# Qualcomm-AI-research/FP8-quantization

Measured on AMD Instinct MI355X. Metric: FP8 quant+dequant Gelems/sec, higher is better.
Workload: dtype f32; 1 GPU; conv1-shaped weights [2097152,3,7,7] fp32 per GPU, per-channel E5M2 quantize+dequantize, fixed ranges from current_minmax (BASELINE config 2, synthetic NxCxKxK scale-up); elements_per_gpu=308281344, parallelism=1 GPU

## Files before the change

### fp8-quantization_amd/csrc/fp8q_device.h

```cpp
#pragma once
#include <hip/hip_runtime.h>
#include <stdint.h>

#include "fp8q_tables.h"

namespace fp8q {

typedef float vf4 __attribute__((ext_vector_type(4)));
typedef float vf4u __attribute__((ext_vector_type(4), aligned(4)));

constexpr int kBlock = 256;
constexpr int kLutMax = 130;

struct QFmt {
    float M;
    float two_E;
    float l_c;
    float qthr;
    int sign_bits;
    int pmax;
};

struct __attribute__((aligned(16))) Chan {
    float maxv, minv, bias;
// ... 91 lines not shown

__device__ __forceinline__ void stage_fast_tab(double *dst)
{
    for (int i = threadIdx.x; i < kFastTabSize; i += kBlock) dst[i] = kFastTab[i];
}

__device__ __forceinline__ float scale_exact(const Chan &c, float ls, float M)
{
    if (__builtin_expect(!(fabsf(c.bias) < __builtin_inff()), 0))
        return c.bias != c.bias ? c.bias : (c.bias > 0.0f ? 0.0f : __builtin_inff());
    const float k = ls - M;
    const float e = k - c.bias;
    const double d = (double)k - c.bias_d;
    const double delta = (double)e - d;
    const double u = delta * 0.69314718055994530942;
    const double t = fma(u, 0.5 * u, u);
    const double s = fma(c.g, t, c.g);
    return (float)ldexp(s, (int)k - c.bi);
}

__device__ __forceinline__ float2 lut_entry(const Chan &c, int p, float M)
{
    if (p == 0) return make_float2(__builtin_nanf(""), __builtin_nanf(""));
    const float k = (float)p - M;
    const float e = k - c.bias;
    float s;
    if ((k - e) == c.bias && c.pthr >= 0.0f)
        s = ldexpf(c.m0, (int)k - c.bi);
    else
        s = scale_exact(c, (float)p, M);
    return make_float2(s, __builtin_amdgcn_rcpf(s));
}

__device__ __forceinline__ void lut_row(float2 *lr, const Chan &c, const QFmt &f)
{
    const float k1 = 1.0f - f.M, kp = (float)f.pmax - f.M;
    const bool lin = c.pthr >= 0.0f && (k1 - (k1 - c.bias)) == c.bias && (kp - (kp - c.bias)) == c.bias;
    lr[0] = make_float2(__builtin_nanf(""), __builtin_nanf(""));
    if (lin) {
        const int j0 = (int)k1 - c.bi - 1;
        for (int p = 1; p <= f.pmax; ++p) {
            const float sc = ldexpf(c.m0, j0 + p);
            lr[p] = make_float2(sc, __builtin_amdgcn_rcpf(sc));
        }
    } else {
        for (int p = 1; p <= f.pmax; ++p) lr[p] = lut_entry(c, p, f.M);
    }
}

__device__ __forceinline__ void lut_part(float2 *lr, const Chan &c, const QFmt &f, int sub, int step)
{
    const float k1 = 1.0f - f.M, kp = (float)f.pmax - f.M;
    const bool lin = c.pthr >= 0.0f && (k1 - (k1 - c.bias)) == c.bias && (kp - (kp - c.bias)) == c.bias;
    if (sub == 0) lr[0] = make_float2(__builtin_nanf(""), __builtin_nanf(""));
    if (lin) {
        const int j0 = (int)k1 - c.bi - 1;
        for (int p = sub ? sub : step; p <= f.pmax; p += step) {
            const float sc = ldexpf(c.m0, j0 + p);
            lr[p] = make_float2(sc, __builtin_amdgcn_rcpf(sc));
        }
    } else {
        for (int p = sub ? sub : step; p <= f.pmax; p += step) lr[p] = lut_entry(c, p, f.M);
    }
}

struct ChanLite {
    float maxv, minv, bias, pthr;
};

__device__ __forceinline__ ChanLite lite(const Chan &c)
{
    ChanLite l;
    l.maxv = c.maxv;
    l.minv = c.minv;
    l.bias = c.bias;
    l.pthr = c.pthr;
    return l;
}

__device__ __forceinline__ ChanLite lite_of(const float4 h)
{
    ChanLite l;
    l.maxv = h.x;
    l.minv = h.y;
    l.bias = h.z;
    l.pthr = h.w;
// ... 41 lines not shown
        any |= rk[j];
    }
    if (__builtin_expect(any, 0)) {
#pragma unroll
        for (int j = 0; j < N; ++j)
            if (rk[j]) y[j] = quant_exact(v[j], c.maxv, c.minv, c.bias, lut, pmaxf);
    }
#pragma unroll
    for (int j = 0; j < N; ++j) v[j] = y[j];
}

__device__ __forceinline__ float quant_one(float x, const ChanLite &c, const float2 *lut, float pmaxf,
                                           float qthr)
{
    bool risky;
    float y = quant_fast(x, c, lut, pmaxf, qthr, risky);
    if (__builtin_expect(risky, 0)) y = quant_exact(x, c.maxv, c.minv, c.bias, lut, pmaxf);
    return y;
}

__device__ __forceinline__ float quant_direct(float x, const Chan &c, float M)
{
    const float xc = __builtin_amdgcn_fmed3f(x, c.minv, c.maxv);
    const float a = fabsf(xc);
    const float v = __builtin_amdgcn_logf(a) + c.bias;
    float fl = floorf(v);
    const float fr = v - fl;
    const bool risky = __builtin_amdgcn_classf(x, 0x90) | (fabsf(fr - 0.5f) > c.pthr) | (c.pthr < 0.0f);
    if (__builtin_expect(risky, 0)) fl = floorf(log2_tab(a, kFastTab) + c.bias);
    const float ls = fmaxf(fl, 1.0f);
    const float s = scale_exact(c, ls, M);
    const float y = rintf(xc / s) * s;
    return (x != x) ? x : y;
}

__device__ __forceinline__ uint32_t code_of_r(float r, float ls, int M, int sign_shift)
{
    if (__builtin_expect(!(fabsf(r) <= (float)(2u << M)), 0)) return 0u;
    const uint32_t ri = (uint32_t)fabsf(r);
    const uint32_t m2 = 1u << M;
    uint32_t e = (uint32_t)ls, f = ri - m2;
    if (ri < m2) {
        e = 0u;
        f = ri;
    } else if (ri == 2u * m2) {
        e += 1u;
        f = 0u;
    }
    const uint32_t sign = sign_shift >= 0 ? ((__float_as_uint(r) >> 31) << sign_shift) : 0u;
    return sign | (e << M) | f;
}

__device__ __forceinline__ uint32_t encode_one(float x, const ChanLite &c, const float2 *lut, float pmaxf,
                                               float qthr, int M, int sign_shift)
{
    const float xc = __builtin_amdgcn_fmed3f(x, c.minv, c.maxv);
    const float v = __builtin_amdgcn_logf(fabsf(xc)) + c.bias;
    float fl = floorf(v);
    const float fr = v - fl;
    float ls = __builtin_amdgcn_fmed3f(fl, 1.0f, pmaxf);
    float2 t = lut[(int)ls];
    float q0 = xc * t.y;
    float r = rintf(q0);
    const bool risky = __builtin_amdgcn_classf(x, 0x93) | (fabsf(fr - 0.5f) > c.pthr) |
                       (fabsf(q0 - r) > qthr) | (c.pthr < 0.0f);
    if (__builtin_expect(risky, 0)) {
// ... 183 lines not shown
```

### fp8-quantization_amd/csrc/fp8q_rows.h

```cpp
#pragma once
#include "fp8q_common.h"

namespace {

constexpr int kModeQuant = 0, kModeFused = 1, kModeMinMax = 2;
constexpr int kModeEncode = 3, kModeDecode = 4;

struct TileArgs {
    int inner;
    int rows;
    int lut_stride;
    int group;
    int coaligned;
    uint32_t magic;
    uint32_t lmagic;
};

__device__ __forceinline__ ChanLite lite_lds(const Chan *c)
{
    const float4 h = *reinterpret_cast<const float4 *>(c);
    ChanLite l;
    l.maxv = h.x;
    l.minv = h.y;
    l.bias = h.z;
    l.pthr = h.w;
    return l;
}

constexpr int kChunkElems = 4096, kChunkGroups = 1024, kFlatMaxCh = 8;
constexpr int kFlatFusedMaxInner = 256;

struct FlatArgs {
    int inner;
    int rpc;
    int nch;
    int lut_stride;
    int group;
    int tail;
    uint32_t magic;
// ... 59 lines not shown
```

### fp8-quantization_amd/csrc/fp8q_rows.hip

```cpp
#include "fp8q_rows.h"

namespace {

template <int MODE, bool LUT, bool NT>
__global__ void __launch_bounds__(kBlock, 4)
k_rows_direct(const float *__restrict__ x, float *__restrict__ y, int64_t C,
              const float *__restrict__ maxval, float *row_min, float *row_max, float *maxval_out,
              QFmt f, TileArgs a, FoldArgs fa)
{
    extern __shared__ __attribute__((aligned(16))) unsigned char smem[];
    const int Rmax = a.rows;
    float *rowmv = reinterpret_cast<float *>(smem);
    float4 *patch = reinterpret_cast<float4 *>(rowmv + ((Rmax + 3) & ~3));
    Chan *chans = reinterpret_cast<Chan *>(patch + Rmax);
    float2 *lut = reinterpret_cast<float2 *>(chans + Rmax);
    const int tid = threadIdx.x;
    constexpr int BS = kBlock;
    const int G = a.group, rpp = BS / G;
    const int sub = tid & (G - 1), slot = tid / G;
    const int inner = a.inner, inner4 = inner & ~3;
    const float pmaxf = (float)f.pmax;
    __shared__ double ftab_lds[kFastTabSize];
    const double *ftab = ftab_lds;
    if (MODE != kModeMinMax)
// ... 90 lines not shown
            for (int j0 = tid; j0 < nvec; j0 += BS * U) {
                vf4 v[U];
#pragma unroll
                for (int u = 0; u < U; ++u)
                    if (j0 + u * BS < nvec) v[u] = ld16u<NT>(xt + head + (j0 + u * BS) * 4);
#pragma unroll
                for (int u = 0; u < U; ++u) {
                    const int j = j0 + u * BS;
                    if (j >= nvec) break;
                    const int o = head + j * 4;
                    const int ch = div_small((uint32_t)o, a.magic);
                    const int b = inner - (o - ch * inner);
                    float e[4] = {v[u].x, v[u].y, v[u].z, v[u].w};
                    if (LUT) {
                        quant_group<4>(e, lite_lds(chans + ch), lut + ch * a.lut_stride, pmaxf, f.qthr);
                    } else {
                        const Chan c = chans[ch];
#pragma unroll
                        for (int q = 0; q < 4; ++q) e[q] = quant_direct(e[q], c, f.M);
                    }
                    if (b < 4) {
                        const float4 pt = patch[ch];
                        e[3] = b == 3 ? pt.x : (b == 2 ? pt.y : pt.z);
                        if (b < 3) e[2] = b == 2 ? pt.x : pt.y;
                        if (b < 2) e[1] = pt.x;
                    }
                    st16u<NT>(yt + o, vf4{e[0], e[1], e[2], e[3]});
                }
            }
        }
    }
}

template <int MODE, bool NT>
__global__ void __launch_bounds__(kBlock, 4)
k_rows_flat(const float *__restrict__ x, float *__restrict__ y, const float *__restrict__ maxval,
            float *row_min, float *row_max, float *maxval_out, QFmt f, FlatArgs a)
{
    extern __shared__ __attribute__((aligned(16))) unsigned char smem[];
    __shared__ double ftab[kFastTabSize];
    const int Rt = a.rpc * a.nch;
    ChunkInfo *cinfo = reinterpret_cast<ChunkInfo *>(smem);
    float4 *patch = reinterpret_cast<float4 *>(cinfo + kFlatMaxCh);
    float4 *chl = patch + Rt;
    float2 *lut = reinterpret_cast<float2 *>(chl + Rt);
    float *rowmv = reinterpret_cast<float *>(lut + Rt * a.lut_stride);
    const int tid = threadIdx.x;
    const int inner = a.inner;
    const int64_t G = gridDim.x;
    const float pmaxf = (float)f.pmax;
    for (int i = tid; i < kFastTabSize; i += kBlock) ftab[i] = kFastTab[i];

    for (int64_t c0 = blockIdx.x; c0 < a.nchunks; c0 += G * a.nch) {
        int nct = 1;
        while (nct < a.nch && c0 + nct * G < a.nchunks) ++nct;
        const int nlr = nct * a.rpc;
        __syncthreads();
        if (tid < nct) {
            const int64_t c = c0 + tid * G;
            const int64_t elo = c * kChunkElems;
            const int64_t rem = a.nvec * 4 - elo;
            ChunkInfo ci;
            ci.len = rem < kChunkElems ? (int)rem : kChunkElems;
            ci.tail = (c == a.nchunks - 1) ? a.tail : 0;
            ci.row_lo = elo / inner;
            ci.phase = (int)(elo - ci.row_lo * inner);
            ci.nrows = (ci.phase + ci.len + ci.tail - 1) / inner + 1;
            ci.pad[0] = ci.pad[1] = 0;
            cinfo[tid] = ci;
        }
        __syncthreads();
// ... 217 lines not shown
}

__device__ __forceinline__ ChunkInfo stage_geometry_next(const ChunkInfo &cur, int64_t cn, uint32_t adv, const FlatArgs &a)
{
    ChunkInfo ci;
    const int64_t elo = cn * kChunkElems;
    const int64_t rem = a.nvec * 4 - elo;
    ci.len = rem < kChunkElems ? (int)rem : kChunkElems;
    ci.tail = (cn == a.nchunks - 1) ? a.tail : 0;
    const uint32_t t = (uint32_t)cur.phase + adv;
    const uint32_t q = (uint32_t)div_small(t, a.magic);
    ci.row_lo = cur.row_lo + q;
    ci.phase = (int)(t - q * (uint32_t)a.inner);
    ci.nrows = div_small((uint32_t)(ci.phase + ci.len + ci.tail - 1), a.magic) + 1;
    ci.pad[0] = ci.nrows * a.inner - ci.phase - ci.len;
    ci.pad[1] = 0;
    return ci;
}

constexpr int kStageU = 4;

template <bool NT>
__device__ __forceinline__ void stage_load_body(const float *x, int64_t c, const FlatArgs &a, vf4 (&v)[kStageU])
{
    const int64_t elo = c * kChunkElems;
    const int64_t rem = a.nvec * 4 - elo;
    const int ng = (rem < kChunkElems ? (int)rem : kChunkElems) >> 2;
    const vf4 *xv = reinterpret_cast<const vf4 *>(x + elo);
#pragma unroll
    for (int u = 0; u < kStageU; ++u)
        if ((int)threadIdx.x + u * kBlock < ng) v[u] = ld16<NT>(xv + threadIdx.x + u * kBlock);
}

__device__ __forceinline__ void stage_load_borders(const float *x, int64_t c, const ChunkInfo &ci, float &bh, float &bt)
{
    const int64_t elo = c * kChunkElems;
    const int tid = threadIdx.x;
    if (tid < ci.phase) bh = x[elo - ci.phase + tid];
    if (tid < ci.pad[0]) bt = x[elo + ci.len + tid];
}

__device__ __forceinline__ void stage_park(float *win, const ChunkInfo &ci, const vf4 (&v)[kStageU], float bh, float bt)
{
    const int tid = threadIdx.x, ng = ci.len >> 2;
#pragma unroll
    for (int u = 0; u < kStageU; ++u)
        if (tid + u * kBlock < ng) *reinterpret_cast<vf4 *>(win + kStagePad + 4 * (tid + u * kBlock)) = v[u];
    if (tid < ci.phase) win[kStagePad - ci.phase + tid] = bh;
    if (tid < ci.pad[0]) win[kStagePad + ci.len + tid] = bt;
}

__device__ __forceinline__ MinMax stage_row_range(const float *wr, bool valid, int inner, int sub, int gs)
{
    const int Gl = 1 << gs, last = inner - 1;
    MinMax m;
    mm_init(m);
    if (valid) {
        for (int j = sub; j < inner; j += 4 * Gl) {
            const float t0 = wr[j], t1 = wr[min(j + Gl, last)], t2 = wr[min(j + 2 * Gl, last)], t3 = wr[min(j + 3 * Gl, last)];
            mm_acc(m, t0);
            mm_acc(m, t1);
            mm_acc(m, t2);
            mm_acc(m, t3);
        }
    }
    if (gs >= 1) mm_dpp<0xB1>(m);
// ... 199 lines not shown
#pragma unroll
    for (int e = 0; e < EPL; ++e) {
        const int i = lane + 64 * e;
        if (i < inner) yr[i] = quant_one(v[e], c, lut[wave], pmaxf, f.qthr);
    }
}

constexpr int64_t kSmallFusedElems = 16384;
constexpr int kSmallFusedInner = 512;

}

int64_t fp8q_direct_max_inner()
{
    static const int v = [] {
        const char *e = getenv("FP8Q_DIRECT_MAX_INNER");
        const int n = e ? atoi(e) : 0;
        return n >= 4 && n <= kDirectMaxInner ? n : 2047;
    }();
    return v;
}

static int64_t flat_nch(const FlatArgs &a, int64_t per_row, int64_t lds_bytes, int64_t max_nch)
{
    int64_t nch = (lds_bytes - (int64_t)kFlatMaxCh * sizeof(ChunkInfo)) / (a.rpc * per_row);
    if (nch > max_nch) nch = max_nch;
    while (nch > 1 && cdiv(a.nchunks, nch) < 1024) --nch;
    return nch;
}

static size_t flat_shmem(const FlatArgs &a, int64_t per_row) { return (size_t)kFlatMaxCh * sizeof(ChunkInfo) + (size_t)a.rpc * a.nch * per_row; }

static int launch_rows_flat(int mode, const float *x, float *y, int64_t C, int64_t inner, const float *maxval,
                            float *row_min, float *row_max, float *maxval_out, const QFmt &f, hipStream_t st)
{
    static const int flat_env = env_int("FP8Q_FLAT", 1);
    if (!flat_env || mode == kModeMinMax || inner < 4) return kNotFlat;
    if ((((uintptr_t)x | (uintptr_t)y) & 15) != 0) return kNotFlat;
    if (mode == kModeFused && (inner > kFlatFusedMaxInner || x == y)) return kNotFlat;
    FlatArgs a = flat_geometry(C, inner, f.pmax + 1);
    const int64_t per_row = flat_per_row(a.lut_stride, mode == kModeFused);
    static const int lds_kb_env = [] {
        const char *e = getenv("FP8Q_FLAT_LDS_KB");
        const int v = e ? atoi(e) : 0;
        return v >= 4 && v <= 120 ? v : 36;
    }();
    static const int nch_env = [] {
        const char *e = getenv("FP8Q_FLAT_NCH");
        const int v = e ? atoi(e) : 0;
        return v >= 1 && v <= kFlatMaxCh ? v : 4;
    }();
    const int64_t nch = flat_nch(a, per_row, (int64_t)lds_kb_env * 1024, nch_env);
    if (nch < 1) return kNotFlat;
    const bool nt = C * inner * 4 >= kNtBytes;
    if (mode == kModeFused) {
        static const int staged_env = env_int("FP8Q_STAGED", 1);
        static const int staged_grid = [] {
            const char *e = getenv("FP8Q_STAGED_GRID");
            const int v = e ? atoi(e) : -1;
            return v >= 0 ? v : kStageGrid;
        }();
        const size_t sh = (size_t)kStageWin * sizeof(float) + (size_t)a.rpc * per_row;
        if (staged_env && sh <= kStageMaxLds) {
            int gs = 0;
            while (gs < 6 && (2 << gs) * a.rpc <= kBlock) ++gs;
            a.group = gs;
            a.nch = 1;
            const int64_t blocks = staged_grid ? balanced_blocks(a.nchunks, staged_grid) : a.nchunks;
            dispatch<true, false>(nt, [&](auto NT) {
                hipLaunchKernelGGL((k_rows_staged<NT()>), dim3((unsigned)blocks), dim3(kBlock), sh, st, x, y, row_min, row_max,
                                   maxval_out, f, a);
            });
            return launch_rc();
        }
    }
    a.nch = (int)nch;
    int G = 1;
    while (G < 64 && (int64_t)G * 24 < inner) G <<= 1;
    a.group = G;
    static const int grid_env = env_int("FP8Q_FLAT_GRID", 0, 0);
    int64_t blocks = cdiv(a.nchunks, a.nch);
    const int64_t grid_cap = grid_env ? grid_env : ((mode == kModeQuant && a.nchunks <= 16384) ? 1024 : 32768);
    if (blocks > grid_cap) blocks = grid_cap;
    dispatch<kModeQuant, kModeFused>(mode, [&](auto MODE) {
        dispatch<true, false>(nt, [&](auto NT) {
            hipLaunchKernelGGL((k_rows_flat<MODE(), NT()>), dim3((unsigned)blocks), dim3(kBlock), flat_shmem(a, per_row), st, x, y,
                               maxval, row_min, row_max, maxval_out, f, a);
        });
    });
    return launch_rc();
}

__attribute__((visibility("hidden"))) int fp8q_codec_flat_launch(bool encode, const void *in, void *out, int64_t C,
                                                                 int64_t inner, const float *maxval, const QFmt &f,
                                                                 int n_bits, hipStream_t st)
{
    const void *fp = encode ? in : (const void *)out;
    const void *cp = encode ? (const void *)out : in;
    if (inner < 4 || inner > fp8q_direct_max_inner() || ((uintptr_t)fp & 15) != 0 || ((uintptr_t)cp & 3) != 0) return kNotFlat;
    FlatArgs a = flat_geometry(C, inner, f.pmax + 1);
    a.n_bits = n_bits;
    const int64_t per_row = flat_per_row(a.lut_stride);
    const int64_t nch = flat_nch(a, per_row, 36 * 1024, 4);
    if (nch < 1) return kNotFlat;
    a.nch = (int)nch;
    a.group = 1;
    int64_t blocks = cdiv(a.nchunks, nch);
    if (blocks > 32768) blocks = 32768;
    const bool nt = C * inner * 4 >= kNtBytes;
    const float *xf = (const float *)in;
    float *yf = (float *)out;
    dispatch<kModeEncode, kModeDecode>(encode ? kModeEncode : kModeDecode, [&](auto MODE) {
        dispatch<true, false>(nt, [&](auto NT) {
            hipLaunchKernelGGL((k_rows_flat<MODE(), NT()>), dim3((unsigned)blocks), dim3(kBlock), flat_shmem(a, per_row), st, xf, yf,
                               maxval, nullptr, nullptr, nullptr, f, a);
        });
    });
    return launch_rc();
}

// ... 54 lines not shown
    const int64_t want = cdiv(C, 1024);
    if (R > want) R = want;
    if (R >= 4) R &= ~(int64_t)3;
    if (R < 1) R = 1;
    a.rows = (int)R;
    a.group = G;
    a.coaligned = (y == nullptr) || ((((uintptr_t)x ^ (uintptr_t)y) & 15) == 0);
    const size_t shmem = (size_t)((R + 3) & ~(int64_t)3) * 4 + (size_t)R * 16 + (size_t)R * sizeof(Chan) +
                         (lut ? (size_t)R * a.lut_stride * sizeof(float2) : 0);
    int64_t blocks = cdiv(C, R);
    static const int mm_blocks_env = env_int("FP8Q_K2_BLOCKS", 65536);
    const int64_t bcap = mode == kModeMinMax ? mm_blocks_env : 2 * kTargetBlocks;
    if (blocks > bcap) blocks = balanced_blocks(blocks, bcap);
    const bool nt = C * inner * 4 >= kNtBytes;
    const dim3 g((unsigned)blocks), b(BSZ);
    auto launch = [&](auto MODE, auto LUT, auto NT) {
        hipLaunchKernelGGL((k_rows_direct<MODE(), LUT(), NT()>), g, b, shmem, st, x, y, C, maxval, row_min, row_max,
                           maxval_out, f, a, fa);
    };
    if (mode == kModeMinMax) {
        launch(Const<kModeMinMax>{}, Const<false>{}, Const<false>{});
    } else {
        dispatch<kModeQuant, kModeFused>(mode, [&](auto MODE) {
            dispatch<true, false>(lut, [&](auto LUT) { dispatch<true, false>(nt, [&](auto NT) { launch(MODE, LUT, NT); }); });
        });
    }
    return launch_rc();
}

extern "C" {

int64_t fp8q_fused_max_inner(void) { return kDirectMaxInner; }

int fp8q_minmax_quantize_f32(const float *x, float *y, int64_t C, int64_t inner, float *row_min,
                             float *row_max, float *maxval_out, float mbits, int n_bits,
                             int sign_bits, fp8q_stream_t stream)
{
    if (C < 0 || inner < 0) return FP8Q_EINVAL;
    QFmt f;
    if (int rc = make_fmt(mbits, n_bits, sign_bits, &f)) return rc;
    if (C == 0 || inner == 0) return FP8Q_OK;
    if (!x || !y) return FP8Q_EINVAL;
    if (inner > kDirectMaxInner) return FP8Q_ETOOLONG;
    if (((uintptr_t)x & 3) != 0 || ((uintptr_t)y & 3) != 0) return FP8Q_EINVAL;
    hipStream_t st = (hipStream_t)stream;
    static const bool small_fused = env_int("FP8Q_SMALL_FUSED", 1) != 0;
    const FoldArgs nofold = {0, 1, 0.0f, 0.0f};
    if (small_fused && C * inner <= kSmallFusedElems && inner <= kSmallFusedInner) {
        dispatch<1, 2, 3, 4, 8>((int)cdiv(inner, 64), [&](auto EPL) {
            hipLaunchKernelGGL(k_small_rows_fused<EPL()>, dim3((unsigned)cdiv(C, kBlock / 64)), dim3(kBlock), 0, st, x, y, C,
                               (int)inner, row_min, row_max, maxval_out, f);
        });
        return launch_rc();
    }
    const int rc = fp8q_launch_rows_reg(true, x, y, C, inner, row_min, row_max, maxval_out, f, nofold, st);
    if (rc != kNotFlat) return rc;
    return fp8q_launch_rows_direct(kModeFused, x, y, C, inner, nullptr, row_min, row_max, maxval_out, f, nofold, st);
}

}
```

### fp8-quantization_amd/fp8q/_lib.py

```python
import ctypes
import os

from . import build as _build

_lib = None

_i64 = ctypes.c_int64
_vp = ctypes.c_void_p
_f = ctypes.c_float
_i = ctypes.c_int



class MseState(ctypes.Structure):
    _fields_ = [("cur_min", _vp), ("cur_max", _vp), ("absmax", _vp), ("grid", _vp), ("mses", _vp), ("maxval", _vp),
                ("xmin", _vp), ("mbits", _vp), ("vote", _vp)]


class MseRouteInfo(ctypes.Structure):
    _fields_ = [("kernel", _i), ("finish", _i), ("nsplit", _i64), ("tiles_per_wg", _i), ("part_wgs", _i), ("slice_min", _i),
                ("moments_threads", _i), ("n_superblocks", _i64), ("top_scan", _i), ("reserved", _i)]


class AffinePre(ctypes.Structure):
    _fields_ = [("x", _vp), ("residual", _vp), ("alpha_beta", _vp), ("N", _i64), ("C", _i64), ("HW", _i64), ("act", _i)]


class MxtRouteInfo(ctypes.Structure):
    _fields_ = [("kernel", _i), ("tile_rows", _i), ("tile_cols", _i), ("nontemporal", _i), ("code_store_bytes", _i),
                ("reserved", _i)]


class TensorDesc(ctypes.Structure):
    _fields_ = [("x", _vp), ("y", _vp), ("maxval", _vp), ("C", _i64), ("inner", _i64), ("n_maxval", _i64),
                ("mbits", _f), ("n_bits", _i), ("sign_bits", _i)]


SIGNATURES = {
    "fp8q_version": (_i, []),
    "fp8q_strerror": (ctypes.c_char_p, [_i]),
    "fp8q_quantize_f32": (_i, [_vp, _vp, _i64, _i64, _vp, _i64, _f, _i, _i, _vp]),
    "fp8q_minmax_workspace_bytes": (ctypes.c_size_t, [_i64, _i64]),
    "fp8q_minmax_f32": (_i, [_vp, _i64, _i64, _vp, _vp, _vp, _i, ctypes.c_double, _i, _vp,
                             ctypes.c_size_t, _vp]),
    "fp8q_minmax_packed_f32": (_i, [_vp, _i64, _i64, _vp, _vp, _vp, _vp, _i, ctypes.c_double, _i, _vp,
                                    ctypes.c_size_t, _vp]),
    "fp8q_ranges_unpack_f32": (_i, [_vp, _i64, _vp, _vp, _vp, _vp]),
    "fp8q_minmax_workspace_check": (_i, [_vp, ctypes.c_size_t, _i, _vp]),
    "fp8q_fused_max_inner": (_i64, []),
    "fp8q_minmax_quantize_f32": (_i, [_vp, _vp, _i64, _i64, _vp, _vp, _vp, _f, _i, _i, _vp]),
    "fp8q_mse_workspace_bytes": (ctypes.c_size_t, [_i64, _i64, _i64, _i]),
    "fp8q_mse_grid_f32": (_i, [_vp, _i64, _i64, _vp, _i64, ctypes.POINTER(_f), _i, _i, _i, _vp, _vp,
                               ctypes.c_size_t, _vp]),
    "fp8q_mse_route": (_i, [_i64, _i64, _i64, ctypes.POINTER(_f), _i, _i, _i, ctypes.POINTER(MseRouteInfo)]),
    "fp8q_mse_linspace_f32": (_i, [_vp, _i64, _i, ctypes.c_double, ctypes.c_double, _vp, _vp]),
    "fp8q_minmax_linspace_f32": (_i, [_vp, _i64, _i64, _vp, _vp, _vp, _vp, _i, ctypes.c_double, ctypes.c_double, _vp,
                                      ctypes.c_size_t, _vp]),
    "fp8q_mse_select_workspace_bytes": (ctypes.c_size_t, [_i64, _i]),
    "fp8q_mse_select_f32": (_i, [_vp, _vp, _i64, _i64, ctypes.POINTER(_f), _i, _i, _vp, _vp, _vp, _vp, _vp,
                                 ctypes.c_size_t, _vp]),
    "fp8q_quantize_dm_f32": (_i, [_vp, _vp, _i64, _i64, _vp, _i64, _vp, _i, _i, _vp]),
    "fp8q_quantize_ds_f32": (_i, [_vp, _vp, _i64, _i64, _vp, _i64, _f, _i, _vp, _vp]),
    "fp8q_sign_fold_u8": (_i, [_vp, _i64, _vp, _vp]),
    "fp8q_quantize_dms_f32": (_i, [_vp, _vp, _i64, _i64, _vp, _i64, _vp, _i, _vp, _vp]),
    "fp8q_mse_calibrate_workspace_bytes": (ctypes.c_size_t, [_i64, _i64, _i64, _i, ctypes.POINTER(ctypes.c_size_t),
                                                             ctypes.POINTER(ctypes.c_size_t)]),
    "fp8q_mse_calibrate_f32": (_i, [_vp, _vp, _i64, _i64, ctypes.POINTER(MseState), _i, _i, ctypes.POINTER(_f), _i, _i, _i,
                                    ctypes.POINTER(AffinePre), _vp, ctypes.c_size_t, _vp, ctypes.c_size_t, _vp, ctypes.c_size_t, _vp]),
    "fp8q_quantize_f64": (_i, [_vp, _vp, _i64, _i64, _vp, _i64, _f, _i, _i, _vp]),
    "fp8q_minmax_f64_workspace_bytes": (ctypes.c_size_t, [_i64, _i64]),
    "fp8q_minmax_f64": (_i, [_vp, _i64, _i64, _vp, _vp, _vp, ctypes.c_size_t, _vp]),
    "fp8q_mse_f64_workspace_bytes": (ctypes.c_size_t, [_i64, _i64, _i64, _i]),
    "fp8q_mse_grid_f64": (_i, [_vp, _i64, _i64, _vp, _i64, ctypes.POINTER(_f), _i, _i, _i, _vp, _i, _vp,
                               ctypes.c_size_t, _vp]),
# ... 111 lines not shown
```

### fp8-quantization_amd/fp8q/ops.py

```python
import torch

from ._lib import Fp8qError, check, lib

FOLD_CURRENT, FOLD_ALL, FOLD_RUNNING = 0, 1, 2

_ws_cache = {}
_ws_retired = []
_mm_ws_bytes = {}


_raw_stream = getattr(torch._C, "_cuda_getCurrentRawStream", None)


def _stream(t):
    if _raw_stream is not None:
        return _raw_stream(t.device.index)
    return torch.cuda.current_stream(t.device).cuda_stream


class _on_device:
    __slots__ = ("idx", "prev")

    def __init__(self, t):
        self.idx = t.device.index
# ... 124 lines not shown
    if fmt is None:
        raise Fp8qError(f"uint8 codes carry no format: pass fmt={hint}")
    return fmt


def _quantize_h16(x, maxval, mbits, n_bits, sign_bits, out, out_dtype):
    if isinstance(mbits, torch.Tensor) or isinstance(sign_bits, torch.Tensor):
        raise Fp8qError("a device-resident mantissa width / sign flag is float32-only: the half-precision lane takes "
                        f"mbits and sign_bits as numbers (x is {x.dtype}; widen it with .float() for that route)")
    dt = _half_out_dtype(x, out, out_dtype)
    _require(x, "x", _HALF)
    _require(maxval, "maxval", like=x)
    maxval = maxval.contiguous().view(-1)
    n_mv = maxval.numel()
    flat = _dense_flat(x) if (n_mv == 1 and out is None) else None
    if flat is not None:
        res = torch.empty_like(x, dtype=dt)
        flat_out = _dense_flat(res) if res.stride() == x.stride() else None
        if flat_out is not None:
            _quantize_h16(flat, maxval, mbits, n_bits, sign_bits, flat_out, None)
            return res
    x = x.contiguous()
    C, inner = _rows(x, n_mv != 1)
    if n_mv != 1 and n_mv != C:
        raise Fp8qError(f"maxval has {n_mv} elements, expected 1 or {C}")
    y = _out(out, x, dtype=dt)
    if x.numel() == 0:
        return y
    with _on_device(x):
        rc = lib().fp8q_quantize_h16(x.data_ptr(), y.data_ptr(), _DT[x.dtype], _DT[dt], C, inner, maxval.data_ptr(), n_mv,
                                     float(mbits), int(n_bits), int(sign_bits), _stream(x))
    check(rc, "fp8q_quantize_h16")
    return y


def quantize(x, maxval, mbits, n_bits=8, sign_bits=1, out=None, out_dtype=None):
    if isinstance(x, torch.Tensor) and x.dtype in _HALF:
        return _quantize_h16(x, maxval, mbits, n_bits, sign_bits, out, out_dtype)
    _require(x, "x", (torch.float32, torch.float64))
    _check_out_dtype(x, out_dtype)
    _require(maxval, "maxval", like=x)
    maxval = maxval.contiguous().view(-1)
    n_mv = maxval.numel()
    flat = _dense_flat(x) if (n_mv == 1 and out is None) else None
    if flat is not None:
        res = torch.empty_like(x)
        flat_out = _dense_flat(res) if res.stride() == x.stride() else None
        if flat_out is not None:
            quantize(flat, maxval, mbits, n_bits, sign_bits, out=flat_out)
            return res
    x = x.contiguous()
    C, inner = _rows(x, n_mv != 1)
    if n_mv != 1 and n_mv != C:
        raise Fp8qError(f"maxval has {n_mv} elements, expected 1 or {C}")
    y = _out(out, x)
    if isinstance(mbits, torch.Tensor) and mbits.is_cuda:
        _require(mbits, "mbits", like=x)
        if mbits.numel() != 1 or x.dtype != torch.float32:
            raise Fp8qError("a device-resident mantissa width must be a 1-element float32 tensor, x float32")
        if isinstance(sign_bits, torch.Tensor):
            _require(sign_bits, "sign_bits", torch.uint8, like=x)
            if sign_bits.numel() != 1:
                raise Fp8qError("a device-resident sign flag must be a 1-element uint8 tensor")
            with _on_device(x):
                rc = lib().fp8q_quantize_dms_f32(x.data_ptr(), y.data_ptr(), C, inner, maxval.data_ptr(), n_mv,
                                                 mbits.data_ptr(), int(n_bits), sign_bits.data_ptr(), _stream(x))
# ... 1531 lines not shown
```

### include/fp8q.h

```cpp
#ifndef FP8Q_H
#define FP8Q_H

#include <stddef.h>
#include <stdint.h>

#ifdef __cplusplus
extern "C" {
#endif

#define FP8Q_VERSION 601

#define FP8Q_OK 0
#define FP8Q_EINVAL (-1)
#define FP8Q_EUNSUPPORTED (-2)
#define FP8Q_EWORKSPACE (-3)
#define FP8Q_ETOOLONG (-4)
#define FP8Q_ETOOMANY (-5)
#define FP8Q_ETIMEDOUT (-6)

#define FP8Q_FOLD_CURRENT 0
#define FP8Q_FOLD_ALL 1
#define FP8Q_FOLD_RUNNING 2


typedef void *fp8q_stream_t;

int fp8q_version(void);
const char *fp8q_strerror(int code);

int fp8q_quantize_f32(const float *x, float *y, int64_t C, int64_t inner, const float *maxval,
                      int64_t n_maxval, float mbits, int n_bits, int sign_bits,
                      fp8q_stream_t stream);

size_t fp8q_minmax_workspace_bytes(int64_t C, int64_t inner);
int fp8q_minmax_f32(const float *x, int64_t C, int64_t inner, float *cur_min, float *cur_max,
                    float *maxval_out, int fold_mode, double momentum, int first, void *ws,
                    size_t ws_bytes, fp8q_stream_t stream);

int fp8q_minmax_packed_f32(const float *x, int64_t C, int64_t inner, float *cur_min, float *cur_max,
                           float *maxval_out, float *packed, int fold_mode, double momentum, int first, void *ws,
                           size_t ws_bytes, fp8q_stream_t stream);
int fp8q_ranges_unpack_f32(const float *packed, int64_t n, float *cur_min, float *cur_max, float *maxval_out,
                           fp8q_stream_t stream);

int fp8q_minmax_workspace_check(void *ws, size_t ws_bytes, int clear, fp8q_stream_t stream);

int64_t fp8q_fused_max_inner(void);
int fp8q_minmax_quantize_f32(const float *x, float *y, int64_t C, int64_t inner, float *row_min,
                             float *row_max, float *maxval_out, float mbits, int n_bits,
                             int sign_bits, fp8q_stream_t stream);

size_t fp8q_mse_workspace_bytes(int64_t C, int64_t inner, int64_t n_cand, int n_m);
int fp8q_mse_grid_f32(const float *x, int64_t C, int64_t inner, const float *grid, int64_t n_cand,
                      const float *mbits_host, int n_m, int n_bits, int sign_bits, float *mses,
                      void *ws, size_t ws_bytes, fp8q_stream_t stream);

typedef struct fp8q_mse_route_info {
    int kernel;
    int finish;
    int64_t nsplit;
    int tiles_per_wg;
    int part_wgs;
    int slice_min;
    int moments_threads;
    int64_t n_superblocks;
// ... 268 lines not shown
```

Before: 756.0 Gelem/s.

## Add table-free flat quantize kernel using per-row scale records instead of LUTs

Adds a quantize path for the flat chunked kernel that stores a compact per-row record (max, bias, base mantissa, exponent offset) in LDS instead of a full per-row scale/reciprocal lookup table. Scales are rebuilt on the fly with ldexp from the record, and rare edge cases fall back to a non-inlined slow path. This shrinks LDS use and removes the table-build work per chunk, which should allow more resident blocks, and it also changes the chunks-per-block count. The old table kernel stays reachable through a new mode behind an environment variable, and a route-query API is added. The cost is some extra per-element ALU work and more register pressure from the larger fast path.

```diff
diff --git a/fp8-quantization_amd/csrc/fp8q_device.h b/fp8-quantization_amd/csrc/fp8q_device.h
--- a/fp8-quantization_amd/csrc/fp8q_device.h
+++ b/fp8-quantization_amd/csrc/fp8q_device.h
@@ -147,10 +147,16 @@
     return make_float2(s, __builtin_amdgcn_rcpf(s));
 }
 
+__device__ __forceinline__ bool chan_lin(const Chan &c, const QFmt &f)
+{
+    const float k1 = 1.0f - f.M, kp = (float)f.pmax - f.M;
+    return c.pthr >= 0.0f && (k1 - (k1 - c.bias)) == c.bias && (kp - (kp - c.bias)) == c.bias;
+}
+
 __device__ __forceinline__ void lut_row(float2 *lr, const Chan &c, const QFmt &f)
 {
-    const float k1 = 1.0f - f.M, kp = (float)f.pmax - f.M;
-    const bool lin = c.pthr >= 0.0f && (k1 - (k1 - c.bias)) == c.bias && (kp - (kp - c.bias)) == c.bias;
+    const float k1 = 1.0f - f.M;
+    const bool lin = chan_lin(c, f);
     lr[0] = make_float2(__builtin_nanf(""), __builtin_nanf(""));
     if (lin) {
         const int j0 = (int)k1 - c.bi - 1;
@@ -165,8 +171,8 @@
 
 __device__ __forceinline__ void lut_part(float2 *lr, const Chan &c, const QFmt &f, int sub, int step)
 {
-    const float k1 = 1.0f - f.M, kp = (float)f.pmax - f.M;
-    const bool lin = c.pthr >= 0.0f && (k1 - (k1 - c.bias)) == c.bias && (kp - (kp - c.bias)) == c.bias;
+    const float k1 = 1.0f - f.M;
+    const bool lin = chan_lin(c, f);
     if (sub == 0) lr[0] = make_float2(__builtin_nanf(""), __builtin_nanf(""));
     if (lin) {
         const int j0 = (int)k1 - c.bi - 1;
@@ -274,6 +280,114 @@
     const float s = scale_exact(c, ls, M);
     const float y = rintf(xc / s) * s;
     return (x != x) ? x : y;
+}
+
+struct __attribute__((aligned(16))) RowRec {
+    float maxv, bias, m0;
+    int j0;
+    float minv, pthr;
+    int bi, pad;
+    double g, bias_d;
+};
+constexpr int kNotLin = INT32_MIN;
+constexpr float kPthrLin = 0.5f - 0x1p-15f;
+
+__device__ __forceinline__ RowRec row_rec(const Chan &c, const QFmt &f)
+{
+    RowRec r;
+    r.maxv = c.maxv;
+    r.bias = c.bias;
+    r.m0 = c.m0;
+    r.j0 = chan_lin(c, f) ? (int)(1.0f - f.M) - c.bi - 1 : kNotLin;
+    r.minv = c.minv;
+    r.pthr = c.pthr;
+    r.bi = c.bi;
+    r.pad = 0;
+    r.g = c.g;
+    r.bias_d = c.bias_d;
+    return r;
+}
+
+struct RowFast {
+    float maxv, bias, m0;
+    int j0;
+};
+
+__device__ __forceinline__ RowFast row_fast(const RowRec *r)
+{
+    const float4 h = *reinterpret_cast<const float4 *>(r);
+    RowFast c;
+    c.maxv = h.x;
+    c.bias = h.y;
+    c.m0 = h.z;
+    c.j0 = __float_as_int(h.w);
+    return c;
+}
+
+__device__ __forceinline__ float quant_fast_rec(float x, const RowFast &c, bool sign, float pmaxf, float qthr, bool &risky)
+{
+    const float xc = __builtin_amdgcn_fmed3f(x, sign ? -c.maxv : 0.0f, c.maxv);
+    const float v = __builtin_amdgcn_logf(fabsf(xc)) + c.bias;
+    const float fl = floorf(v);
+    const float fr = v - fl;
+    const float ls = __builtin_amdgcn_fmed3f(fl, 1.0f, pmaxf);
+    const float s = ldexpf(c.m0, c.j0 + (int)ls);
+    const float q0 = xc * __builtin_amdgcn_rcpf(s);
+    const float r = rintf(q0);
+    risky = __builtin_amdgcn_classf(x, 0x93) | (fabsf(fr - 0.5f) > kPthrLin) | (fabsf(q0 - r) > qthr) | (c.j0 == kNotLin);
+    return r * s;
+}
+
+__device__ __noinline__ float quant_slow_rec(float x, const RowRec *r, float pmaxf, float M)
+{
+    if (r->j0 != kNotLin) {
+        if (x != x) return x;
+        const float xc = __builtin_amdgcn_fmed3f(x, r->minv, r->maxv);
+        float ls = floorf(log2_tab(fabsf(xc), kFastTab) + r->bias);
+        ls = __builtin_amdgcn_fmed3f(ls, 1.0f, pmaxf);
+        const float s = ldexpf(r->m0, r->j0 + (int)ls);
+        return rintf(xc / s) * s;
+    }
+    Chan c;
+    c.maxv = r->maxv;
+    c.minv = r->minv;
+    c.bias = r->bias;
+    c.pthr = r->pthr;
+    c.g = r->g;
+    c.bias_d = r->bias_d;
+    c.m0 = r->m0;
+    c.bi = r->bi;
+    c.bf = c.pad1 = 0.0f;
+    return quant_direct(x, c, M);
+}
+
+template <int N>
+__device__ __forceinline__ void quant_group_rec(float (&v)[N], const RowRec *const (&rec)[N], const QFmt &f)
+{
+    const float pmaxf = (float)f.pmax;
+    float y[N];
+    bool rk[N];
+    bool any = false;
+#pragma unroll
+    for (int j = 0; j < N; ++j) {
+        y[j] = quant_fast_rec(v[j], row_fast(rec[j]), f.sign_bits == 1, pmaxf, f.qthr, rk[j]);
+        any |= rk[j];
+    }
+    if (__builtin_expect(any, 0)) {
+#pragma unroll
+        for (int j = 0; j < N; ++j)
+            if (rk[j]) y[j] = quant_slow_rec(v[j], rec[j], pmaxf, f.M);
+    }
+#pragma unroll
+    for (int j = 0; j < N; ++j) v[j] = y[j];
+}
+
+__device__ __forceinline__ float quant_one_rec(float x, const RowRec *rec, const QFmt &f)
+{
+    float v[1] = {x};
+    const RowRec *const r[1] = {rec};
+    quant_group_rec<1>(v, r, f);
+    return v[0];
 }
 
 __device__ __forceinline__ uint32_t code_of_r(float r, float ls, int M, int sign_shift)
diff --git a/fp8-quantization_amd/csrc/fp8q_rows.h b/fp8-quantization_amd/csrc/fp8q_rows.h
--- a/fp8-quantization_amd/csrc/fp8q_rows.h
+++ b/fp8-quantization_amd/csrc/fp8q_rows.h
@@ -5,6 +5,7 @@
 
 constexpr int kModeQuant = 0, kModeFused = 1, kModeMinMax = 2;
 constexpr int kModeEncode = 3, kModeDecode = 4;
+constexpr int kModeQuantLut = 5;
 
 struct TileArgs {
     int inner;
diff --git a/fp8-quantization_amd/csrc/fp8q_rows.hip b/fp8-quantization_amd/csrc/fp8q_rows.hip
--- a/fp8-quantization_amd/csrc/fp8q_rows.hip
+++ b/fp8-quantization_amd/csrc/fp8q_rows.hip
@@ -146,11 +146,22 @@
     }
 }
 
+constexpr int kFreeBlocksPerCU = 4;
+constexpr int kFreeNch = 2, kFreeMaxNch = 4;
+
+template <bool NT>
+__device__ __forceinline__ void rows_flat_tablefree(const float *__restrict__ x, float *__restrict__ y,
+                                                    const float *__restrict__ maxval, const QFmt &f, const FlatArgs &a);
+
 template <int MODE, bool NT>
-__global__ void __launch_bounds__(kBlock, 4)
+__global__ void __launch_bounds__(kBlock, MODE == kModeQuant ? kFreeBlocksPerCU : 4)
 k_rows_flat(const float *__restrict__ x, float *__restrict__ y, const float *__restrict__ maxval,
             float *row_min, float *row_max, float *maxval_out, QFmt f, FlatArgs a)
 {
+    if constexpr (MODE == kModeQuant) {
+        rows_flat_tablefree<NT>(x, y, maxval, f, a);
+        return;
+    }
     extern __shared__ __attribute__((aligned(16))) unsigned char smem[];
     __shared__ double ftab[kFastTabSize];
     const int Rt = a.rpc * a.nch;
@@ -434,6 +445,91 @@
         if ((int)threadIdx.x + u * kBlock < ng) v[u] = ld16<NT>(xv + threadIdx.x + u * kBlock);
 }
 
+template <bool NT>
+__device__ __forceinline__ void rows_flat_tablefree(const float *__restrict__ x, float *__restrict__ y,
+                                                    const float *__restrict__ maxval, const QFmt &f, const FlatArgs &a)
+{
+    extern __shared__ __attribute__((aligned(16))) unsigned char smem[];
+    __shared__ double ftab[kFastTabSize];
+    __shared__ ChunkInfo cinfo[kFlatMaxCh];
+    RowRec *recs = reinterpret_cast<RowRec *>(smem);
+    const int tid = threadIdx.x;
+    const int inner = a.inner;
+    const int64_t G = gridDim.x;
+    constexpr int U = kStageU, T =(kFastTabSize + kBlock - 1) / kBlock;
+    bool staged = false;
+    for (int64_t c0 = blockIdx.x; c0 < a.nchunks; c0 += G * a.nch) {
+        int nct = 1;
+        while (nct < a.nch && c0 + nct * G < a.nchunks) ++nct;
+        const int nlr = nct * a.rpc;
+        ChunkInfo ci;
+        int ic, r;
+        auto pair_of = [&](int lr) -> bool {
+            ic = div_small((uint32_t)lr, a.rmagic);
+            r = lr - ic * a.rpc;
+            if (lr >= nlr) return false;
+            ci = stage_geometry(c0 + ic * G, a);
+            return r < ci.nrows;
+        };
+        bool mine = pair_of(tid);
+        float mv = 0.0f;
+        if (mine) mv = maxval[ci.row_lo + r];
+        double t[T];
+        if (!staged) {
+#pragma unroll
+            for (int k = 0; k < T; ++k)
+                if (tid + k * kBlock < kFastTabSize) t[k] = kFastTab[tid + k * kBlock];
+        }
+        vf4 v[U];
+        stage_load_body<NT>(x, c0, a, v);
+        if (!staged) {
+#pragma unroll
+            for (int k = 0; k < T; ++k)
+                if (tid + k * kBlock < kFastTabSize) ftab[tid + k * kBlock] = t[k];
+            staged = true;
+        }
+        __syncthreads();
+        for (int lr = tid; lr < nlr; lr += kBlock) {
+            if (lr != tid) {
+                mine = pair_of(lr);
+                if (mine) mv = maxval[ci.row_lo + r];
+            }
+            if (mine) {
+                recs[lr] = row_rec(make_chan_fast(mv, f, ftab), f);
+                if (r == 0) cinfo[ic] = ci;
+            }
+        }
+        __syncthreads();
+        if (tid < cinfo[nct - 1].tail) {
+            const ChunkInfo cl = cinfo[nct - 1];
+            const int e = cl.len + tid;
+            const int lr = (nct - 1) * a.rpc + div_small((uint32_t)(cl.phase + e), a.magic);
+            const int64_t at = (c0 + (nct - 1) * G) * kChunkElems + e;
+            y[at] = quant_one_rec(x[at], recs + lr, f);
+        }
+        for (int i = 0; i < nct; ++i) {
+            const int64_t c = c0 + i * G;
+            if (i > 0) stage_load_body<NT>(x, c, a, v);
+            const int phase = cinfo[i].phase, ng = cinfo[i].len >> 2;
+            vf4 *yv = reinterpret_cast<vf4 *>(y + c * kChunkElems);
+            const RowRec *rc = recs + i * a.rpc;
+#pragma unroll
+            for (int u = 0; u < U; ++u) {
+                const int q = tid + u * kBlock;
+                if (q >= ng) break;
+                const int o = phase + 4 * q;
+                const int lrow = div_small((uint32_t)o, a.magic);
+                const int b = inner - (o - lrow * inner);
+                const RowRec *r0 = rc + lrow, *r1 = r0 + 1;
+                const RowRec *const rj[4] = {r0, b > 1 ? r0 : r1, b > 2 ? r0 : r1, b > 3 ? r0 : r1};
+                float e[4] = {v[u].x, v[u].y, v[u].z, v[u].w};
+                quant_group_rec<4>(e, rj, f);
+                st16<NT>(yv + q, vf4{e[0], e[1], e[2], e[3]});
+            }
+        }
+    }
+}
+
 __device__ __forceinline__ void stage_load_borders(const float *x, int64_t c, const ChunkInfo &ci, float &bh, float &bt)
 {
     const int64_t elo = c * kChunkElems;
@@ -699,7 +795,8 @@
 static size_t flat_shmem(const FlatArgs &a, int64_t per_row) { return (size_t)kFlatMaxCh * sizeof(ChunkInfo) + (size_t)a.rpc * a.nch * per_row; }
 
 static int launch_rows_flat(int mode, const float *x, float *y, int64_t C, int64_t inner, const float *maxval,
-                            float *row_min, float *row_max, float *maxval_out, const QFmt &f, hipStream_t st)
+                            float *row_min, float *row_max, float *maxval_out, const QFmt &f, hipStream_t st,
+                            fp8q_k1_route_info *route = nullptr)
 {
     static const int flat_env = env_int("FP8Q_FLAT", 1);
     if (!flat_env || mode == kModeMinMax || inner < 4) return kNotFlat;
@@ -741,18 +838,40 @@
             return launch_rc();
         }
     }
+    static const int k1_tables_env = env_int("FP8Q_K1_TABLES", 0);
+    const bool tablefree = mode == kModeQuant && !k1_tables_env;
     a.nch = (int)nch;
+    if (tablefree) {
+        static const int free_nch = [] {
+            const char *e = getenv("FP8Q_FLAT_NCH");
+            const int v = e ? atoi(e) : 0;
+            return v >= 1 && v <= kFreeMaxNch ? v : kFreeNch;
+        }();
+        a.nch = free_nch;
+        while (a.nch > 1 && cdiv(a.nchunks, a.nch) < 1024) --a.nch;
+    }
     int G = 1;
     while (G < 64 && (int64_t)G * 24 < inner) G <<= 1;
     a.group = G;
     static const int grid_env = env_int("FP8Q_FLAT_GRID", 0, 0);
     int64_t blocks = cdiv(a.nchunks, a.nch);
-    const int64_t grid_cap = grid_env ? grid_env : ((mode == kModeQuant && a.nchunks <= 16384) ? 1024 : 32768);
+    const bool resident = mode == kModeQuant && a.nchunks <= 16384;
+    const int64_t grid_cap = grid_env ? grid_env : (resident ? 1024 : 32768);
     if (blocks > grid_cap) blocks = grid_cap;
-    dispatch<kModeQuant, kModeFused>(mode, [&](auto MODE) {
+    const size_t shmem = tablefree ? (size_t)a.rpc * a.nch * sizeof(RowRec) : flat_shmem(a, per_row);
+    if (route) {
+        route->kernel = tablefree ? FP8Q_K1_FLAT : FP8Q_K1_FLAT_TABLES;
+        route->chunks_per_block = a.nch;
+        route->nontemporal = nt;
+        route->resident_grid = resident;
+        route->blocks = blocks;
+        route->lds_bytes = (int64_t)shmem;
+        return FP8Q_OK;
+    }
+    dispatch<kModeQuant, kModeQuantLut, kModeFused>(mode == kModeQuant && !tablefree ? kModeQuantLut : mode, [&](auto MODE) {
         dispatch<true, false>(nt, [&](auto NT) {
-            hipLaunchKernelGGL((k_rows_flat<MODE(), NT()>), dim3((unsigned)blocks), dim3(kBlock), flat_shmem(a, per_row), st, x, y,
-                               maxval, row_min, row_max, maxval_out, f, a);
+            hipLaunchKernelGGL((k_rows_flat<MODE(), NT()>), dim3((unsigned)blocks), dim3(kBlock), shmem, st, x, y, maxval,
+                               row_min, row_max, maxval_out, f, a);
         });
     });
     return launch_rc();
@@ -873,6 +992,23 @@
 
 int64_t fp8q_fused_max_inner(void) { return kDirectMaxInner; }
 
+int fp8q_k1_route(int64_t C, int64_t inner, float mbits, int n_bits, int sign_bits, int aligned16, fp8q_k1_route_info *info)
+{
+    if (C <= 0 || inner <= 0 || !info) return FP8Q_EINVAL;
+    QFmt f;
+    if (int rc = make_fmt(mbits, n_bits, sign_bits, &f)) return rc;
+    fp8q_k1_route_info r = {};
+    r.kernel = FP8Q_K1_ROWS;
+    if (inner <= fp8q_direct_max_inner()) {
+        r.kernel = FP8Q_K1_DIRECT;
+        float *p = reinterpret_cast<float *>((uintptr_t)(aligned16 ? 16 : 4));
+        const int rc = launch_rows_flat(kModeQuant, p, p, C, inner, nullptr, nullptr, nullptr, nullptr, f, nullptr, &r);
+        if (rc != kNotFlat && rc != FP8Q_OK) return rc;
+    }
+    *info = r;
+    return FP8Q_OK;
+}
+
 int fp8q_minmax_quantize_f32(const float *x, float *y, int64_t C, int64_t inner, float *row_min,
                              float *row_max, float *maxval_out, float mbits, int n_bits,
                              int sign_bits, fp8q_stream_t stream)
diff --git a/fp8-quantization_amd/fp8q/_lib.py b/fp8-quantization_amd/fp8q/_lib.py
--- a/fp8-quantization_amd/fp8q/_lib.py
+++ b/fp8-quantization_amd/fp8q/_lib.py
@@ -31,6 +31,11 @@
                 ("reserved", _i)]
 
 
+class K1RouteInfo(ctypes.Structure):
+    _fields_ = [("kernel", _i), ("chunks_per_block", _i), ("nontemporal", _i), ("resident_grid", _i), ("blocks", _i64),
+                ("lds_bytes", _i64)]
+
+
 class TensorDesc(ctypes.Structure):
     _fields_ = [("x", _vp), ("y", _vp), ("maxval", _vp), ("C", _i64), ("inner", _i64), ("n_maxval", _i64),
                 ("mbits", _f), ("n_bits", _i), ("sign_bits", _i)]
@@ -40,6 +45,7 @@
     "fp8q_version": (_i, []),
     "fp8q_strerror": (ctypes.c_char_p, [_i]),
     "fp8q_quantize_f32": (_i, [_vp, _vp, _i64, _i64, _vp, _i64, _f, _i, _i, _vp]),
+    "fp8q_k1_route": (_i, [_i64, _i64, _f, _i, _i, _i, ctypes.POINTER(K1RouteInfo)]),
     "fp8q_minmax_workspace_bytes": (ctypes.c_size_t, [_i64, _i64]),
     "fp8q_minmax_f32": (_i, [_vp, _i64, _i64, _vp, _vp, _vp, _i, ctypes.c_double, _i, _vp,
                              ctypes.c_size_t, _vp]),
diff --git a/fp8-quantization_amd/fp8q/ops.py b/fp8-quantization_amd/fp8q/ops.py
--- a/fp8-quantization_amd/fp8q/ops.py
+++ b/fp8-quantization_amd/fp8q/ops.py
@@ -180,6 +180,20 @@
                                      float(mbits), int(n_bits), int(sign_bits), _stream(x))
     check(rc, "fp8q_quantize_h16")
     return y
+
+
+_K1_KERNELS = ("rows", "direct", "flat_tables", "flat")
+
+
+def k1_route(C, inner, mbits, n_bits=8, sign_bits=1, aligned16=True):
+    from ._lib import K1RouteInfo
+    import ctypes
+    info = K1RouteInfo()
+    check(lib().fp8q_k1_route(int(C), int(inner), float(mbits), int(n_bits), int(sign_bits), int(bool(aligned16)),
+                              ctypes.byref(info)), "fp8q_k1_route")
+    return {"kernel": _K1_KERNELS[info.kernel], "chunks_per_block": info.chunks_per_block,
+            "nontemporal": bool(info.nontemporal), "resident_grid": bool(info.resident_grid), "blocks": info.blocks,
+            "lds_bytes": info.lds_bytes}
 
 
 def quantize(x, maxval, mbits, n_bits=8, sign_bits=1, out=None, out_dtype=None):
diff --git a/include/fp8q.h b/include/fp8q.h
--- a/include/fp8q.h
+++ b/include/fp8q.h
@@ -31,6 +31,20 @@
 int fp8q_quantize_f32(const float *x, float *y, int64_t C, int64_t inner, const float *maxval,
                       int64_t n_maxval, float mbits, int n_bits, int sign_bits,
                       fp8q_stream_t stream);
+
+#define FP8Q_K1_ROWS 0
+#define FP8Q_K1_DIRECT 1
+#define FP8Q_K1_FLAT_TABLES 2
+#define FP8Q_K1_FLAT 3
+typedef struct fp8q_k1_route_info {
+    int kernel;
+    int chunks_per_block;
+    int nontemporal;
+    int resident_grid;
+    int64_t blocks;
+    int64_t lds_bytes;
+} fp8q_k1_route_info;
+int fp8q_k1_route(int64_t C, int64_t inner, float mbits, int n_bits, int sign_bits, int aligned16, fp8q_k1_route_info *info);
 
 size_t fp8q_minmax_workspace_bytes(int64_t C, int64_t inner);
 int fp8q_minmax_f32(const float *x, int64_t C, int64_t inner, float *cur_min, float *cur_max,
```

Result: no change. 761.3 Gelem/s (median of 4 runs) (+0.7%).
